# shehryar-malik/icrl

Hardware: AMD Instinct MI355X
Metric: env-steps/sec (ICRL outer loop, HCWithPos-v0) (higher is better)
Workload: dtype f32

## Files before the change

icrl_amd/_lib.py:

```python
import ctypes
import os

_HERE = os.path.dirname(os.path.abspath(__file__))
LIB_PATH = os.environ.get("ICRL_HIP_LIB") or os.path.join(_HERE, "lib", "libicrl_hip.so")

_lib = None
PPO_SPLIT_BYTES = 2560 * 1024

c_void_p, c_int, c_double, c_float = ctypes.c_void_p, ctypes.c_int, ctypes.c_double, ctypes.c_float

SIGNATURES = {
    "icrl_abi_version": [],
    "icrl_last_error": [],
    "icrl_clear_error": [],
    "icrl_gae_dual": [c_void_p] * 12 + [c_int, c_int] + [c_double] * 4 + [c_void_p],
    "icrl_gae_dual_ex": [c_void_p] * 12 + [c_int, c_int] + [c_double] * 4 + [c_int, c_void_p],
    "icrl_gae_dual_ws": [c_void_p] * 12 + [c_int, c_int] + [c_double] * 4 + [c_int, c_void_p, ctypes.c_longlong, c_void_p],
    "icrl_gae_dual_ws_bytes": [c_int, c_int],
    "icrl_policy_prepare": [c_void_p, c_void_p],
    "icrl_costnet_prepare": [c_void_p, c_void_p],
    "icrl_policy_forward": [c_void_p, c_void_p, c_void_p, c_int, c_int] + [c_void_p] * 8,
    "icrl_policy_evaluate": [c_void_p, c_void_p, c_void_p, c_int] + [c_void_p] * 5,
    "icrl_sample_episodes": [c_void_p] * 6 + [c_int] * 4 + [c_void_p, c_int] + [c_void_p] * 6,
    "icrl_cost_mlp_forward": [c_void_p, c_void_p, c_void_p, c_int, c_void_p, c_void_p],
# ... 16 lines not shown
    "icrl_ppo_lag_train": [c_void_p] * 11,
    "icrl_ppo_generic_row_floats": [c_void_p],
    "icrl_cn_prepare": [c_void_p, c_void_p, c_void_p, c_int, c_void_p, c_void_p],
    "icrl_cn_train_work_floats": [c_int, c_int, c_int, c_int],
    "icrl_cn_train": [c_void_p] * 6 + [c_int, c_int, c_void_p, c_void_p, c_int, c_void_p, c_void_p, c_void_p, c_void_p],
    "icrl_debug_rollout_profile": [c_void_p],
    "icrl_debug_rollout_profile_wide": [c_void_p],
    "icrl_debug_rollout_trace_wide": [c_void_p, c_int],
    "icrl_debug_stream_ref": [c_void_p] * 9 + [c_int, c_int, c_int, c_void_p],
    "icrl_minibatch_gather": [c_void_p, c_void_p, c_int] + [c_void_p] * 10,
    "icrl_adv_stats": [c_void_p, c_void_p, c_int, c_void_p, c_void_p],
    "icrl_ppo_lag_loss_fwd_bwd": [c_void_p] * 13 + [c_int] + [c_void_p] * 6,
    "icrl_clip_adam_step": [c_void_p] * 5 + [ctypes.c_longlong, c_void_p, c_void_p, c_void_p, c_void_p],
    "icrl_explained_variance": [c_void_p] * 4 + [ctypes.c_longlong, c_void_p, c_void_p, c_void_p],
    "icrl_dual_step": [c_void_p, c_void_p, c_void_p, c_float, c_float, c_float, c_float, c_void_p, c_void_p],
    "icrl_buffer_add": [c_void_p, c_int] + [c_void_p] * 13,
    "icrl_is_weights": [c_void_p, c_void_p, c_int, c_void_p, c_int, c_float, c_int, c_void_p, c_void_p, c_void_p, c_void_p],
    "icrl_cn_loss_fwd_bwd": [c_void_p, c_void_p, c_void_p, c_int, c_int, c_float, c_float, c_int, c_void_p, c_void_p, c_void_p, c_void_p],
    "icrl_cn_train_minibatch": [c_void_p] * 6 + [c_int, c_int, c_void_p, c_void_p, c_int, c_void_p, c_void_p, c_int, c_void_p,
                                c_void_p, c_void_p],
    "icrl_rollout_collect_batch": [c_int, c_void_p, c_void_p, c_void_p] + [c_double] * 4 + [c_int, c_void_p, ctypes.c_longlong, c_void_p],
    "icrl_gae_dual_batch": [c_int, c_void_p, c_int, c_int] + [c_double] * 4 + [c_void_p, ctypes.c_longlong, c_void_p],
    "icrl_sample_episodes_batch": [c_int, c_void_p, c_void_p, c_void_p] + [c_int] * 4 + [c_void_p, ctypes.c_longlong, c_void_p],
    "icrl_cn_train_batch": [c_int, c_void_p, c_void_p, ctypes.c_longlong, c_void_p],
    "icrl_ppo_lag_train_batch": [c_int, c_void_p, c_void_p, ctypes.c_longlong, c_void_p],
}
BATCH_ARGS_BYTES = 1024
RESTYPES = {"icrl_cn_train_work_floats": ctypes.c_size_t, "icrl_monitor_ws_bytes": ctypes.c_size_t, "icrl_host_step_ws_bytes": ctypes.c_size_t, "icrl_gae_dual_ws_bytes": ctypes.c_size_t, "icrl_last_error": ctypes.c_char_p, "icrl_clear_error": None}


class HipExtensionMissing(RuntimeError):
    pass


def lib():
    global _lib
    if _lib is None:
        import torch
        if not os.path.exists(LIB_PATH):
            raise HipExtensionMissing(
                f"{LIB_PATH} not built: run `python -c 'import __graft_entry__ as g; g.build()'` "
                "(or `make -C icrl_amd/csrc`). icrl_amd has no CPU fallback.")
        _lib = ctypes.CDLL(LIB_PATH)
        for name, argtypes in SIGNATURES.items():
            fn = getattr(_lib, name)
            fn.argtypes = argtypes
            fn.restype = RESTYPES.get(name, c_int)
    return _lib


byref = ctypes.byref
# ... 22 lines not shown
```

icrl_amd/csrc/rollout.hip:

```cpp
#include <stdio.h>
#include <stdlib.h>

#include "common.h"
#include "cost_fn.h"
#include "generic.h"

namespace icrl {

__global__ void policy_transpose_kernel(PolLayout L, const float* __restrict__ p, float* __restrict__ pt) {
  for (int i = blockIdx.x * blockDim.x + threadIdx.x; i < L.n; i += gridDim.x * blockDim.x) {
    int dst = i;
    for (int w = 0; w < 3; ++w) {
      if (i >= L.W1[w] && i < L.b1[w]) { int r = i - L.W1[w]; int j = r / L.O, k = r % L.O; dst = L.W1[w] + k * L.H1 + j; }
      if (i >= L.W2[w] && i < L.b2[w]) { int r = i - L.W2[w]; int j = r / L.H1, k = r % L.H1; dst = L.W2[w] + k * L.H2 + j; }
    }
    if (i >= L.Wa && i < L.ba) { int r = i - L.Wa; int a = r / L.H2, j = r % L.H2; dst = L.Wa + j * L.A + a; }
    pt[dst] = p[i];
  }
}

__global__ void costnet_transpose_kernel(CnLayout L, const float* __restrict__ p, float* __restrict__ pt) {
  for (int i = blockIdx.x * blockDim.x + threadIdx.x; i < L.n; i += gridDim.x * blockDim.x) {
    int dst = i;
    if (i >= L.W0 && i < L.b0) { int r = i - L.W0; int j = r / L.in, k = r % L.in; dst = L.W0 + k * L.H1 + j; }
// ... 2686 lines not shown
    if (i == 0) e.t_ep[n] = 0;
  }
}

struct SampleArgs {
  icrl_env_t env;
  icrl_norm_t nm;
  PolLayout pl;
  const float* PT;
  int pt_in_lds;
  const float* noise;
  const float* alow;
  const float* ahigh;
  int episodes_per_stream, rows_per_stream, deterministic, do_reset;
  const int* stream_row0;
  int total_rows;
  double* orig_obs;
  double* obs;
  float* actions;
  double* ep_rewards;
  int* ep_lengths;
};

template <int OCT>
__device__ __forceinline__ void sample_episodes_body(const SampleArgs& a) {
  __shared__ ActShared sh;
  PolRegs<OCT> R;
  load_pol_regs<OCT>(a.pl, a.PT, R);
  __shared__ int s_done;
  __shared__ double s_rew;
  __shared__ double Bl[MAX_OBS * MAX_ACT];
  __shared__ float noise_s[MAX_ACT], alow_s[MAX_ACT], ahigh_s[MAX_ACT];
  const int n = blockIdx.x, tid = threadIdx.x, lane = tid & 63;
  const int w = __builtin_amdgcn_readfirstlane(tid >> 6);
  const int O = a.pl.O, A = a.pl.A;
  const int AS = a.pl.discrete ? 1 : A;
  icrl_env_t env = a.env; globalize(env);
  const float* const noise_g = as_global(a.noise);
  float* const actions_g = as_global(a.actions);
  double* const orig_obs_g = as_global(a.orig_obs);
  double* const obs_g = as_global(a.obs);
  const int norm_obs = a.nm.norm_obs, deterministic = a.deterministic;
  const double clip_obs = a.nm.clip_obs;
  for (int i = tid; i < O * a.env.act_dim; i += 192) Bl[i] = a.env.B[i];
  env.B = Bl;
  const bool has_box = a.alow != nullptr && a.ahigh != nullptr;
  if (tid < MAX_ACT) { alow_s[tid] = (has_box && tid < A) ? a.alow[tid] : 0.f; ahigh_s[tid] = (has_box && tid < A) ? a.ahigh[tid] : 0.f; }
  const uint32_t e_key = a.env.key[n];
  uint32_t e_ctr = a.env.step_count[n];
  int e_tep = a.env.t_ep[n];
  double n_mean = 0.0, n_den = 1.0;
  if (tid < O && a.nm.norm_obs) { n_mean = a.nm.obs_mean[tid]; n_den = sqrt(a.nm.obs_var[tid] + a.nm.epsilon); }
  for (int i = tid; i < MAX_OBS; i += 192) sh.x[i] = 0.f;
  if (tid < O) {
    double v = a.env.s[(size_t)n * O + tid];
    if (a.do_reset) v = env_reset_value(a.env, e_key, e_ctr, tid);
    sh.s_new[tid] = v;
  }
  if (a.do_reset) e_tep = 0;
  __syncthreads();
  size_t row = a.stream_row0 != nullptr ? (size_t)a.stream_row0[n] : (size_t)n * a.rows_per_stream;
  const size_t row_end = a.stream_row0 != nullptr ? (size_t)a.total_rows : row + a.rows_per_stream;
  float noise_reg = (noise_g != nullptr && tid < AS) ? noise_g[row * AS + tid] : 0.f;
  for (int ep = 0; ep < a.episodes_per_stream; ++ep) {
    double ep_rew = 0.0;
    int ep_len = 0;
    while (true) {
      if (tid < O) {
        const double raw = sh.s_new[tid];
        double o = raw;
        if (norm_obs) o = fmin(fmax((raw - n_mean) / n_den, -clip_obs), clip_obs);
        sh.s_old[tid] = raw;
        sh.x[tid] = (float)o;
      }
      if (noise_g != nullptr && tid < AS) {
        noise_s[tid] = noise_reg;
        if (row + 1 < row_end) noise_reg = noise_g[(row + 1) * AS + tid];
      }
      __syncthreads();
      policy_forward_block<OCT>(a.pl, R, sh, noise_g ? noise_s : nullptr, deterministic || noise_g == nullptr,
                                has_box ? alow_s : nullptr, has_box ? ahigh_s : nullptr);
      __syncthreads();
      const bool in_rows = row < row_end;
      if (w == 0) {
        double rew; int done;
        env_step_wave(env, n, sh.s_old, sh.act_clip, e_key, e_ctr, e_tep, sh.s_new, rew, done);
        if (lane == 0) { s_done = done; s_rew = rew; }
        if (lane < AS && in_rows) actions_g[row * AS + lane] = sh.act_clip[lane];
      }
      __syncthreads();
      if (tid < O && in_rows) {
        const double raw = sh.s_new[tid];
        double o = raw;
        if (norm_obs) o = fmin(fmax((raw - n_mean) / n_den, -clip_obs), clip_obs);
        orig_obs_g[row * O + tid] = raw;
        obs_g[row * O + tid] = o;
      }
      ep_rew += s_rew;
      ++ep_len;
      ++row;
      const int done = s_done;
      __syncthreads();
      if (done) break;
    }
    if (tid == 0) { a.ep_rewards[(size_t)n * a.episodes_per_stream + ep] = ep_rew; a.ep_lengths[(size_t)n * a.episodes_per_stream + ep] = ep_len; }
  }
}

template <int OCT>
__global__ void __launch_bounds__(192) sample_episodes_kernel(SampleArgs a) {
  sample_episodes_body<OCT>(a);
}

template <int OCT>
__global__ void __launch_bounds__(192) sample_episodes_batch_kernel(const SampleArgs* __restrict__ runs) {
  __shared__ SampleArgs a;
  {
    const unsigned* src = reinterpret_cast<const unsigned*>(runs + blockIdx.y);
    unsigned* dst = reinterpret_cast<unsigned*>(&a);
    for (unsigned i = threadIdx.x; i < sizeof(SampleArgs) / 4; i += 192) dst[i] = src[i];
  }
  __syncthreads();
  sample_episodes_body<OCT>(a);
}

struct HostStepArgs {
  ActStepArgs act;
  icrl_norm_t nm;
  icrl_host_step_t hs;
  int N;
};

__host__ __device__ inline size_t host_copy_doubles(int N, int O) { return (size_t)2 * O + 7 + (size_t)3 * N; }
struct HostCopy {
  double *mean, *var, *count, *ret_stats, *cost_stats, *ret, *cost_ret, *cost;
  __device__ HostCopy(double* base, int N, int O)
      : mean(base), var(base + O), count(base + 2 * O), ret_stats(base + 2 * O + 1), cost_stats(base + 2 * O + 4),
        ret(base + 2 * O + 7), cost_ret(base + 2 * O + 7 + N), cost(base + 2 * O + 7 + 2 * N) {}
};

template <int OCT, int CIT>
__global__ void __launch_bounds__(256) host_step_kernel(HostStepArgs h, int k) {
  __shared__ ActShared sh;
  __shared__ double vec[2][128], dev2[2][128], ret_s[128], cret_s[128], rawr_s[128];
  __shared__ float rawc_s[128];
  __shared__ double dens[2];
// ... 462 lines not shown
                                          void* args_ws, long long args_ws_bytes, void* stream) {
  static_assert(sizeof(SampleArgs) <= ICRL_BATCH_ARGS_BYTES, "ICRL_BATCH_ARGS_BYTES");
  if (n_runs < 1 || n_runs > 65535) return fail("icrl_sample_episodes_batch: n_runs = %d (1..65535)", n_runs);
  if (args_ws == nullptr || args_ws_bytes < (long long)n_runs * ICRL_BATCH_ARGS_BYTES)
    return fail("icrl_sample_episodes_batch: args_ws holds %lld B, %d runs need %lld", args_ws_bytes, n_runs, (long long)n_runs * ICRL_BATCH_ARGS_BYTES);
  hipStream_t s = (hipStream_t)stream;
  SampleArgs* d_args = (SampleArgs*)args_ws;
  const icrl_sample_job_t& j0 = jobs[0];
  for (int r = 0; r < n_runs; ++r) {
    const icrl_sample_job_t& j = jobs[r];
    if (j.env->n_envs != j0.env->n_envs || j.env->obs_dim != j0.env->obs_dim || j.pol->act_dim != j0.pol->act_dim ||
        j.pol->discrete != j0.pol->discrete || j.env->max_steps != j0.env->max_steps)
      return fail("icrl_sample_episodes_batch: run %d differs from run 0 in a shape (streams / obs / act / discrete / max_steps)", r);
    SampleArgs a;
    const int bad = make_sample_args(j.env, j.nm, j.pol, j.noise, action_low, action_high, episodes_per_stream, rows_per_stream,
                                     deterministic, do_reset, j.stream_row0, j.total_rows, j.orig_obs, j.obs, j.actions, j.ep_rewards,
                                     j.ep_lengths, a);
    if (bad) return bad;
    const int e = put_args(a, d_args + r, s);
    if (e) return e;
  }
  if (j0.pol->obs_dim <= 32) hipLaunchKernelGGL(sample_episodes_batch_kernel<2>, dim3(j0.env->n_envs, n_runs), dim3(192), 0, s, d_args);
  else hipLaunchKernelGGL(sample_episodes_batch_kernel<8>, dim3(j0.env->n_envs, n_runs), dim3(192), 0, s, d_args);
  return (int)hipGetLastError();
}

extern "C" int icrl_cost_fn_rows(const icrl_cost_fn_t* cf, const double* obs, const float* acs, int N, float* cost, void* stream) {
  if (cf == nullptr || cf->n_hidden != ICRL_COST_FN) return fail("icrl_cost_fn_rows: not an analytic cost descriptor (n_hidden must be ICRL_COST_FN)");
  if (int e = cost_fn_check("icrl_cost_fn_rows", cf, 0, 0, -1)) return e;
  if (N <= 0 || cost == nullptr) return fail("icrl_cost_fn_rows: N = %d rows, cost = %p", N, (void*)cost);
  const bool wall = cf->kind == ICRL_COST_WALL_BEHIND || cf->kind == ICRL_COST_WALL_INFRONT || cf->kind == ICRL_COST_WALL_BOTH;
  if ((wall && obs == nullptr) || ((cf->kind == ICRL_COST_TORQUE || cf->kind == ICRL_COST_ACTION_EQUALS) && acs == nullptr))
    return fail("icrl_cost_fn_rows: cost kind %d reads the %s, which is NULL", cf->kind, wall ? "observations" : "actions");
  const int grid = (N + 255) / 256 < 1024 ? (N + 255) / 256 : 1024;
  hipLaunchKernelGGL(cost_fn_rows_kernel, dim3(grid), dim3(256), 0, (hipStream_t)stream, *cf, obs, acs, N, cost);
  return (int)hipGetLastError();
}

extern "C" int icrl_cost_mlp_forward(const icrl_costnet_t* cn, const double* obs, const float* acs, int N, float* cost,
                                     void* stream) {
  if (const icrl_cost_fn_t* cf = as_cost_fn(cn)) return icrl_cost_fn_rows(cf, obs, acs, N, cost, stream);
  if (N <= 0) return fail("cost forward: N = %d rows", N);
  if (costnet_is_wide(cn)) return launch_cn_cost_rows(cn, obs, acs, N, cost, 0, (hipStream_t)stream);
  if (!cn_ok(cn)) return bad_cn("cost forward", cn);
  CnLayout L = make_cn_layout(cn->in_dim, cn->n_hidden, cn->h1, cn->h2);
  if (cn->in_dim <= 32) hipLaunchKernelGGL(cost_forward_kernel<2>, dim3(N), dim3(64), 0, (hipStream_t)stream, *cn, L, obs, acs, N, cost, 0);
// ... 672 lines not shown
```

icrl_amd/icrl.py:

```python
import argparse
import json
import os
import sys
import time
import types

import numpy as np
import torch

from . import distributed as D, logger, utils
from .constraint_net import ConstraintNet
from .ppo_lag import PPOLagrangian
from .true_constraint_net import get_true_cost_function, mean_cost, null_cost
from .vec_env import VecNormalize, sync_envs_normalization
from . import envs, spaces


def setup(config):
    rank, world = getattr(config, "rank", 0), getattr(config, "world_size", 1)
    dev = config.device if str(config.device).startswith("cuda") else "cuda"
    envs.import_modules(getattr(config, "env_module", None))
    train_env = utils.make_train_env(env_id=config.train_env_id, save_dir=config.save_dir, use_cost_wrapper=True,
                                     base_seed=config.seed, num_threads=config.num_threads,
                                     normalize_obs=not config.dont_normalize_obs, normalize_reward=not config.dont_normalize_reward,
# ... 83 lines not shown
    st["rms_prev"] = D.allreduce_state([pol.params, pol.exp_avg, pol.exp_avg_sq, cn.params, cn.exp_avg, cn.exp_avg_sq],
                                       st["rms_list"], st["rms_prev"], st["world"], scalars=scal, force_collective=force)
    pol.prepare(); cn.prepare()
    if ev is not None:
        ev[1].record(); st["sync_events"].append(ev); st["sync_host_ms"].append(1e3 * (time.perf_counter() - t0))


def outer_iteration(st, itr):
    config, rank, world = st["config"], st["rank"], st["world"]
    train_env, sampling_env, eval_env, constraint_net = st["train_env"], st["sampling_env"], st["eval_env"], st["constraint_net"]
    if config.reset_policy and itr != 0:
        old_agent = st["agent"]
        st["agent"] = st["create_nominal_agent"]()
        if hasattr(old_agent, "_train_ws"):
            st["agent"]._train_ws = old_agent._train_ws
    nominal_agent = st["agent"]
    current_progress_remaining = 1 - float(itr) / float(config.n_iters)
    nominal_agent.learn(total_timesteps=config.forward_timesteps, cost_function="cost")
    forward_metrics = dict(logger.Logger.CURRENT.name_to_value)
    st["timesteps"] += nominal_agent.num_timesteps
    sync_envs_normalization(train_env, sampling_env)
    streams = getattr(config, "streams", None)
    A = 1 if nominal_agent.policy.discrete else nominal_agent.policy.act_dim
    orig_observations, observations, actions, rewards, lengths = utils.sample_from_agent(
        nominal_agent, sampling_env, config.expert_rollouts,
        noise=None if streams is None else streams.sample_noise(config.expert_rollouts * sampling_env.unwrapped.max_steps, A))
    mean, var = None, None
    if config.cn_normalize:
        mean, var = sampling_env.obs_rms.mean, sampling_env.obs_rms.var
    cn_perms = None
    if constraint_net.batch_size is not None and streams is not None and hasattr(streams, "cn_permutations"):
        cn_perms = streams.cn_permutations(config.backward_iters, min(int(orig_observations.shape[0]), int(np.asarray(constraint_net.expert_obs).shape[0])))
    backward_metrics = constraint_net.train(config.backward_iters, orig_observations, actions, lengths, mean, var,
                                            current_progress_remaining, perms=cn_perms)
    train_env.set_cost_function(constraint_net.cost_function)
    synchronise(st)
    average_true_cost = mean_cost(st["true_cost_function"], orig_observations, actions)
    samples_behind = float((orig_observations[..., 0] < -3).double().mean().item())
    samples_infront = float((orig_observations[..., 0] > 3).double().mean().item())
    sync_envs_normalization(train_env, eval_env)
    average_true_reward, std_true_reward = utils.evaluate_policy(
        nominal_agent, eval_env, n_eval_episodes=10, deterministic=False,
        noise=None if streams is None else streams.eval_noise(10 * eval_env.unwrapped.max_steps, A))
    forward_kl = reverse_kl = float("nan")
    if st["expert_agent"] is not None:
        forward_kl = utils.compute_kl(nominal_agent, st["d_expert_obs"], st["d_expert_acs"], st["expert_agent"])
        reverse_kl = utils.compute_kl(st["expert_agent"], orig_observations, actions, nominal_agent)
    best = st["best"]
    if config.save_dir and itr % config.save_every == 0 and rank == 0:
        path = os.path.join(config.save_dir, f"models/icrl_{itr}_itrs")
        os.makedirs(path, exist_ok=True)
        nominal_agent.save(os.path.join(path, "nominal_agent"))
        torch.save(nominal_agent.policy.state_dict(), os.path.join(path, "nominal_agent_policy.pth"))
        constraint_net.save(os.path.join(path, "cn.pt"))
        train_env.save(os.path.join(path, f"{itr}_train_env_stats.pkl"))
    if average_true_reward > best["reward"] and config.save_dir and rank == 0:
        nominal_agent.save(os.path.join(config.save_dir, "best_nominal_model"))
        torch.save(nominal_agent.policy.state_dict(), os.path.join(config.save_dir, "best_nominal_model_policy.pth"))
        constraint_net.save(os.path.join(config.save_dir, "best_cn_model.pt"))
        train_env.save(os.path.join(config.save_dir, "train_env_stats.pkl"))
    best["reward"] = max(best["reward"], average_true_reward)
    best["cost"] = min(best["cost"], average_true_cost)
    best["fkl"] = min(best["fkl"], forward_kl) if forward_kl == forward_kl else best["fkl"]
    best["rkl"] = min(best["rkl"], reverse_kl) if reverse_kl == reverse_kl else best["rkl"]
    metrics = {"time(m)": (time.time() - st["start_time"]) / 60, "iteration": itr, "timesteps": st["timesteps"],
               "true/reward": average_true_reward, "true/reward_std": std_true_reward, "true/cost": average_true_cost,
# ... 105 lines not shown
```

icrl_amd/structs.py:

```python
import ctypes as C

i32, f64, vp = C.c_int32, C.c_double, C.c_void_p


class EnvT(C.Structure):
    _fields_ = [("n_envs", i32), ("obs_dim", i32), ("act_dim", i32), ("max_steps", i32), ("reward_form", i32),
                ("wall_terminate", i32), ("broken", i32), ("_pad", i32),
                ("B", vp), ("s", vp), ("t_ep", vp), ("step_count", vp), ("key", vp)]


class NormT(C.Structure):
    _fields_ = [("training", i32), ("norm_obs", i32), ("norm_reward", i32), ("norm_cost", i32),
                ("clip_obs", f64), ("clip_reward", f64), ("clip_cost", f64), ("reward_gamma", f64), ("cost_gamma", f64),
                ("epsilon", f64),
                ("obs_mean", vp), ("obs_var", vp), ("obs_count", vp), ("ret_stats", vp), ("cost_stats", vp),
                ("ret", vp), ("cost_ret", vp)]


class PolicyT(C.Structure):
    _fields_ = [("obs_dim", i32), ("act_dim", i32), ("h1", i32), ("h2", i32), ("discrete", i32), ("n_params", i32),
                ("params", vp), ("params_t", vp), ("arch", vp)]


class CostNetT(C.Structure):
# ... 47 lines not shown
                ("adam_eps", C.c_float)]


class CnHyperT(C.Structure):
    _fields_ = [("iterations", i32), ("importance_sampling", i32), ("per_step", i32), ("gail", i32),
                ("reg_coeff", C.c_float), ("eps", C.c_float), ("target_kl_old_new", C.c_float), ("target_kl_new_old", C.c_float),
                ("lr", C.c_float), ("adam_beta1", C.c_float), ("adam_beta2", C.c_float), ("adam_eps", C.c_float)]


class RolloutJobT(C.Structure):
    _fields_ = [("env", vp), ("nm", vp), ("pol", vp), ("cn", vp), ("buf", vp), ("ag", vp), ("noise", vp)]


class GaeJobT(C.Structure):
    _fields_ = [(k, vp) for k in ("rewards", "costs", "reward_values", "cost_values", "dones", "last_v_r", "last_v_c", "last_dones",
                                  "adv_r", "adv_c", "ret_r", "ret_c", "ws")] + [("ws_bytes", C.c_longlong)]


class SampleJobT(C.Structure):
    _fields_ = ([(k, vp) for k in ("env", "nm", "pol", "noise", "stream_row0")] + [("total_rows", i32), ("_pad", i32)] +
                [(k, vp) for k in ("orig_obs", "obs", "actions", "ep_rewards", "ep_lengths")])


class CnTrainJobT(C.Structure):
    _fields_ = [("cn", vp), ("exp_avg", vp), ("exp_avg_sq", vp), ("adam_step", vp), ("nominal", vp), ("expert", vp), ("Nn", i32), ("Ne", i32),
                ("ep_offsets", vp), ("row_episode", vp), ("n_ep", i32), ("_pad", i32), ("hp", vp), ("work", vp), ("metrics", vp)]


class PpoTrainJobT(C.Structure):
    _fields_ = [(k, vp) for k in ("pol", "exp_avg", "exp_avg_sq", "adam_step", "buf", "perms", "nu", "hp", "stats", "sync_ws")]


def addr(struct):
    return C.addressof(struct) if struct is not None else None


def p(t):
    if t is None:
        return None
    assert t.is_contiguous()
    return t.data_ptr()

GAE_WS_BYTES = 256 * (256 * 8 + 4) + 64
```

icrl_amd/utils.py:

```python
import io
import os
import pickle
import types
import zipfile

import numpy as np
import torch

from . import _lib, spaces
from .policies import ActorTwoCriticsPolicy
from .structs import EnvT, HostEpisodeT, p
from . import envs
from .vec_env import ENV_IDS, DummyVecEnv, HipSynthVecEnv, HostVecEnv, SubprocVecEnv, VecCostWrapper, VecNormalize, VecNormalizeWithCost


def make_vec_env(env_id, n_envs, seed, device="cuda", env_index_offset=0, dummy_vec_env=False):
    if env_id in ENV_IDS:
        return HipSynthVecEnv.make(env_id, n_envs, seed, device, env_index_offset=env_index_offset)
    fns = [envs.spec(env_id)] * n_envs
    cls = DummyVecEnv if dummy_vec_env else SubprocVecEnv
    venv = cls(fns, device=device, env_index_offset=env_index_offset)
    venv.seed(seed)
    return venv


def make_train_env(env_id, save_dir, use_cost_wrapper, base_seed=0, num_threads=1, normalize_obs=True, normalize_reward=True,
                   normalize_cost=True, env_index_offset=0, device="cuda", **kwargs):
    import random
    random.seed(base_seed); np.random.seed(base_seed); torch.manual_seed(base_seed)
    env = make_vec_env(env_id, num_threads, base_seed, device, env_index_offset, dummy_vec_env=kwargs.pop("dummy_vec_env", False))
    if use_cost_wrapper:
        env = VecCostWrapper(env)
    if normalize_reward and normalize_cost:
        assert all(key in kwargs for key in ["cost_info_str", "reward_gamma", "cost_gamma"])
# ... 93 lines not shown
            lengths = self.out["ep_lengths"].cpu().numpy()
        lengths = np.asarray(lengths).astype(np.int64)
        if self.n_streams > 1:
            implied = np.concatenate([[0], np.cumsum(lengths)[:-1]])
            if not np.array_equal(implied, self.starts):
                if self.passes >= self.MAX_PASSES:
                    self.n_streams = 1
                    self.starts = np.zeros(1, np.int64)
                else:
                    self.starts = implied
                return False
        senv, env, dev = self.senv, self.env, self.dev
        total = int(lengths.sum())
        senv.step_count.fill_(int(np.uint32((self.base + total) & 0xFFFFFFFF).view(np.int32)))
        senv.s.copy_(self.st["s"][-1:]); senv.t_ep.zero_()
        env.old_obs = senv.s
        self.lengths = lengths
        self.keep = None if total == self.rows else total
        return True

    def rows_of(self, name):
        x = self.out[name]
        return x if self.keep is None else x[:self.keep]


class SteppedEpisodeRun:

    def __init__(self, agent, env, n_episodes, deterministic, noise):
        assert env.num_envs == 1, "You must pass only one environment when using this function"
        pol, senv = agent.policy, env.unwrapped
        dev, max_steps = senv.device, senv.max_steps
        A = 1 if pol.discrete else pol.act_dim
        rows = n_episodes * max_steps
        if noise is None and not deterministic:
            noise = torch.rand(rows, device=dev) if pol.discrete else torch.randn(rows, A, device=dev)
        if noise is not None:
            noise = torch.as_tensor(noise, device=dev).float().reshape(rows, -1).contiguous()
        was_training = env.training
        env.training = False
        try:
            orig, obs_l, acts, ep_rewards, lengths = [], [], [], [], []
            k, obs = 0, env.reset()
            for _ in range(n_episodes):
                done, ep_r, ep_l = False, 0.0, 0
                while not done:
                    actions, _, _, _ = pol.forward(obs, deterministic=deterministic, noise=None if noise is None else noise[k:k + 1])
# ... 92 lines not shown
                done = bool(d[0])
                launch(k, int(not (done and ep == n_episodes - 1)))
            ep_rewards.append(ep_r); lengths.append(ep_l)
        last_raw = out["orig_obs"][k - 1:k]
        henv.s.copy_(last_raw)
        nenv.old_obs, nenv.old_reward = last_raw.clone(), torch.full((1,), rew, dtype=torch.float64, device=dev)
        nenv.ret.zero_()
        if cw is not None:
            cw.previous_obs = last_raw.clone()
            cw.actions = out["actions"][k - 1:k].clone()
            if cw.cost_function is not None:
                nenv.cost_ret.zero_()
        out["ep_rewards"] = torch.as_tensor(np.asarray(ep_rewards, np.float64), device=dev)
        out["ep_lengths"] = torch.as_tensor(np.asarray(lengths, np.int32), device=dev)
        self.out, self._keepalive = out, (noise, lo, hi)
        self.lengths = np.asarray(lengths, np.int64)
        self.keep = None if k == rows else k

    def rows_of(self, name):
        x = self.out[name]
        return x if self.keep is None else x[:self.keep]


def _run_episodes(agent, env, n_episodes, deterministic, noise, parallel):
    if isinstance(env.unwrapped, HostVecEnv):
        if env.unwrapped.max_steps is None:
            raise ValueError("sampling / evaluation over a host env needs its episode limit: register it with max_episode_steps "
                             "(or give the env spec.max_episode_steps / _max_episode_steps)")
        if host_episodes_ok(agent, env):
            return HostEpisodeRun(agent, env, n_episodes, deterministic, noise)
        return SteppedEpisodeRun(agent, env, n_episodes, deterministic, noise)
    run = EpisodeRun(agent, env, n_episodes, deterministic, noise, parallel).prepare()
    run.launch()
    while not run.finish():
        run.prepare().launch()
    return run


def sample_from_agent(agent, env, rollouts, noise=None, parallel=True):
    return sample_result(_run_episodes(agent, env, rollouts, False, noise, parallel))


def sample_result(run, ep_rewards=None):
    return (run.rows_of("orig_obs"), run.rows_of("obs"), run.rows_of("actions"),
            run.out["ep_rewards"].cpu().numpy() if ep_rewards is None else np.asarray(ep_rewards), run.lengths)


def evaluate_policy(model, env, n_eval_episodes=10, deterministic=True, render=False, callback=None, reward_threshold=None,
                    return_episode_rewards=False, noise=None):
    run = _run_episodes(model, env, n_eval_episodes, deterministic, noise, parallel=False)
    return evaluate_result(run, None, reward_threshold, return_episode_rewards)


def evaluate_result(run, ep_rewards=None, reward_threshold=None, return_episode_rewards=False):
    ep_rewards = run.out["ep_rewards"].cpu().numpy() if ep_rewards is None else np.asarray(ep_rewards)
    if return_episode_rewards:
        return list(ep_rewards), list(run.lengths)
    mean_reward, std_reward = float(np.mean(ep_rewards)), float(np.std(ep_rewards))
    if reward_threshold is not None:
        assert mean_reward > reward_threshold
    return mean_reward, std_reward


def compute_kl(agent_2, observations, actions, agent_1=None):
    return float(compute_kl_device(agent_2, observations, actions, agent_1).item())


def compute_kl_device(agent_2, observations, actions, agent_1=None):
    kl = -agent_2.policy.evaluate_actions(observations, actions)[1].reshape(-1)
    if agent_1 is not None:
        kl = kl + agent_1.policy.evaluate_actions(observations, actions)[1].reshape(-1)
    return kl.sum() / kl.shape[0]

# ... 121 lines not shown
```

include/icrl_hip.h:

```cpp
#ifndef ICRL_HIP_H
#define ICRL_HIP_H

#include <stdint.h>

#ifdef __cplusplus
extern "C" {
#endif


typedef struct {
  int32_t n_envs, obs_dim, act_dim, max_steps;
  int32_t reward_form;
  int32_t wall_terminate;
  int32_t broken;
  int32_t _pad;
  const double* B;
  double* s;
  int32_t* t_ep;
  uint32_t* step_count;
  const uint32_t* key;
} icrl_env_t;

typedef struct {
  int32_t training, norm_obs, norm_reward, norm_cost;
// ... 247 lines not shown
  void* ws;
  long long ws_bytes;
} icrl_gae_job_t;
int icrl_gae_dual_batch(int n_runs, const icrl_gae_job_t* jobs, int T, int N, double reward_gamma, double reward_gae_lambda,
                        double cost_gamma, double cost_gae_lambda, void* args_ws, long long args_ws_bytes, void* stream);

typedef struct {
  const icrl_env_t* env;
  const icrl_norm_t* nm;
  const icrl_policy_t* pol;
  const float* noise;
  const int32_t* stream_row0;
  int32_t total_rows, _pad;
  double *orig_obs, *obs;
  float* actions;
  double* ep_rewards;
  int32_t* ep_lengths;
} icrl_sample_job_t;
int icrl_sample_episodes_batch(int n_runs, const icrl_sample_job_t* jobs, const float* action_low, const float* action_high,
                               int episodes_per_stream, int rows_per_stream, int deterministic, int do_reset,
                               void* args_ws, long long args_ws_bytes, void* stream);

typedef struct {
  const icrl_costnet_t* cn;
  float *exp_avg, *exp_avg_sq;
  int32_t* adam_step;
  const float *nominal, *expert;
  int32_t Nn, Ne;
  const int32_t *ep_offsets, *row_episode;
  int32_t n_ep, _pad;
  const icrl_cn_hyper_t* hp;
  float *work, *metrics;
} icrl_cn_train_job_t;
int icrl_cn_train_batch(int n_runs, const icrl_cn_train_job_t* jobs, void* args_ws, long long args_ws_bytes, void* stream);

typedef struct {
  const icrl_policy_t* pol;
  float *exp_avg, *exp_avg_sq;
  int32_t* adam_step;
  const icrl_buffer_t* buf;
  const int32_t* perms;
  const float* nu;
  const icrl_ppo_hyper_t* hp;
  float* stats;
  void* sync_ws;
} icrl_ppo_train_job_t;
// ... 51 lines not shown
```

Before: 936,200.

## Run sequential episodes speculatively in parallel with chained predecessor validation

Adds a chained episode sampler that launches one workgroup per episode. Each workgroup speculatively guesses its starting RNG counter and row offset, then re-runs if its predecessor publishes a different end position, so episodes that used to run one after another can overlap. Finished rows are compacted from per-stream slots into the contiguous output. Expert sampling and evaluation are also fused into a single launch. The cost is extra spin-waiting, possible redundant recomputation, a requirement that every workgroup be co-resident, and a new workspace allocation on each call.

Result: faster. 947,300, median of 6 (+1.2%).

```diff
diff --git a/icrl_amd/_lib.py b/icrl_amd/_lib.py
--- a/icrl_amd/_lib.py
+++ b/icrl_amd/_lib.py
@@ -62,11 +62,13 @@
     "icrl_rollout_collect_batch": [c_int, c_void_p, c_void_p, c_void_p] + [c_double] * 4 + [c_int, c_void_p, ctypes.c_longlong, c_void_p],
     "icrl_gae_dual_batch": [c_int, c_void_p, c_int, c_int] + [c_double] * 4 + [c_void_p, ctypes.c_longlong, c_void_p],
     "icrl_sample_episodes_batch": [c_int, c_void_p, c_void_p, c_void_p] + [c_int] * 4 + [c_void_p, ctypes.c_longlong, c_void_p],
+    "icrl_sample_episodes_chain_ws_bytes": [c_int, c_void_p],
+    "icrl_sample_episodes_chain": [c_int, c_void_p, c_void_p, c_void_p, c_int, c_void_p, ctypes.c_longlong, c_void_p, ctypes.c_longlong, c_void_p],
     "icrl_cn_train_batch": [c_int, c_void_p, c_void_p, ctypes.c_longlong, c_void_p],
     "icrl_ppo_lag_train_batch": [c_int, c_void_p, c_void_p, ctypes.c_longlong, c_void_p],
 }
 BATCH_ARGS_BYTES = 1024
-RESTYPES = {"icrl_cn_train_work_floats": ctypes.c_size_t, "icrl_monitor_ws_bytes": ctypes.c_size_t, "icrl_host_step_ws_bytes": ctypes.c_size_t, "icrl_gae_dual_ws_bytes": ctypes.c_size_t, "icrl_last_error": ctypes.c_char_p, "icrl_clear_error": None}
+RESTYPES = {"icrl_cn_train_work_floats": ctypes.c_size_t, "icrl_monitor_ws_bytes": ctypes.c_size_t, "icrl_host_step_ws_bytes": ctypes.c_size_t, "icrl_gae_dual_ws_bytes": ctypes.c_size_t, "icrl_sample_episodes_chain_ws_bytes": ctypes.c_size_t, "icrl_last_error": ctypes.c_char_p, "icrl_clear_error": None}
 
 
 class HipExtensionMissing(RuntimeError):
diff --git a/icrl_amd/csrc/rollout.hip b/icrl_amd/csrc/rollout.hip
--- a/icrl_amd/csrc/rollout.hip
+++ b/icrl_amd/csrc/rollout.hip
@@ -2732,13 +2732,27 @@
   int* ep_lengths;
 };
 
-template <int OCT>
-__device__ __forceinline__ void sample_episodes_body(const SampleArgs& a) {
+struct ChainArgs {
+  SampleArgs s;
+  unsigned* next_start;
+  unsigned* status;
+  int* exec_steps;
+  double* slot_orig;
+  double* slot_obs;
+  float* slot_act;
+  const int* base_count;
+  int fixed_len, n_streams;
+};
+constexpr unsigned CHAIN_UNSET = 0xFFFFFFFEu;
+
+template <int OCT, bool CHAIN = false>
+__device__ __forceinline__ void sample_episodes_body(const SampleArgs& a, const ChainArgs* c = nullptr) {
   __shared__ ActShared sh;
   PolRegs<OCT> R;
   load_pol_regs<OCT>(a.pl, a.PT, R);
   __shared__ int s_done;
   __shared__ double s_rew;
+  __shared__ unsigned s_word;
   __shared__ double Bl[MAX_OBS * MAX_ACT];
   __shared__ float noise_s[MAX_ACT], alow_s[MAX_ACT], ahigh_s[MAX_ACT];
   const int n = blockIdx.x, tid = threadIdx.x, lane = tid & 63;
@@ -2747,9 +2761,9 @@
   const int AS = a.pl.discrete ? 1 : A;
   icrl_env_t env = a.env; globalize(env);
   const float* const noise_g = as_global(a.noise);
-  float* const actions_g = as_global(a.actions);
-  double* const orig_obs_g = as_global(a.orig_obs);
-  double* const obs_g = as_global(a.obs);
+  float* const actions_g = as_global(CHAIN ? c->slot_act : a.actions);
+  double* const orig_obs_g = as_global(CHAIN ? c->slot_orig : a.orig_obs);
+  double* const obs_g = as_global(CHAIN ? c->slot_obs : a.obs);
   const int norm_obs = a.nm.norm_obs, deterministic = a.deterministic;
   const double clip_obs = a.nm.clip_obs;
   for (int i = tid; i < O * a.env.act_dim; i += 192) Bl[i] = a.env.B[i];
@@ -2762,20 +2776,38 @@
   double n_mean = 0.0, n_den = 1.0;
   if (tid < O && a.nm.norm_obs) { n_mean = a.nm.obs_mean[tid]; n_den = sqrt(a.nm.obs_var[tid] + a.nm.epsilon); }
   for (int i = tid; i < MAX_OBS; i += 192) sh.x[i] = 0.f;
+  const int max_steps = a.env.max_steps;
+  unsigned* const words = CHAIN ? as_global(c->next_start) : nullptr;
+  const uint32_t base = CHAIN ? (uint32_t)as_global(c->base_count)[0] : 0u;
+  const size_t slot0 = CHAIN ? (size_t)n * max_steps : 0;
+  unsigned pos = CHAIN ? (unsigned)n * (unsigned)max_steps : 0u;
+  bool validated = !CHAIN || n == 0 || c->fixed_len != 0;
+  int executed = 0;
+  bool again;
+  do {
+  again = false;
+  if (CHAIN) {
+    __syncthreads();
+    e_ctr = base + pos;
+    if (n > 0 || a.do_reset) e_tep = 0;
+    if (tid == 0 && !c->fixed_len) xstore(words + n, (pos + (unsigned)max_steps) << 1);
+  }
   if (tid < O) {
     double v = a.env.s[(size_t)n * O + tid];
-    if (a.do_reset) v = env_reset_value(a.env, e_key, e_ctr, tid);
+    if (a.do_reset || (CHAIN && n > 0)) v = env_reset_value(a.env, e_key, e_ctr, tid);
     sh.s_new[tid] = v;
   }
-  if (a.do_reset) e_tep = 0;
+  if (!CHAIN && a.do_reset) e_tep = 0;
   __syncthreads();
-  size_t row = a.stream_row0 != nullptr ? (size_t)a.stream_row0[n] : (size_t)n * a.rows_per_stream;
-  const size_t row_end = a.stream_row0 != nullptr ? (size_t)a.total_rows : row + a.rows_per_stream;
+  size_t row = CHAIN ? (size_t)pos : a.stream_row0 != nullptr ? (size_t)a.stream_row0[n] : (size_t)n * a.rows_per_stream;
+  const size_t row_end = (CHAIN || a.stream_row0 != nullptr) ? (size_t)a.total_rows : row + a.rows_per_stream;
   float noise_reg = (noise_g != nullptr && tid < AS) ? noise_g[row * AS + tid] : 0.f;
   for (int ep = 0; ep < a.episodes_per_stream; ++ep) {
     double ep_rew = 0.0;
     int ep_len = 0;
     while (true) {
+      unsigned word = CHAIN_UNSET;
+      if (CHAIN && !validated && tid == 128) word = xload(words + n - 1);
       if (tid < O) {
         const double raw = sh.s_new[tid];
         double o = raw;
@@ -2791,30 +2823,76 @@
       policy_forward_block<OCT>(a.pl, R, sh, noise_g ? noise_s : nullptr, deterministic || noise_g == nullptr,
                                 has_box ? alow_s : nullptr, has_box ? ahigh_s : nullptr);
       __syncthreads();
-      const bool in_rows = row < row_end;
+      const bool in_rows = CHAIN || row < row_end;
+      const size_t orow = CHAIN ? slot0 + (size_t)ep_len : row;
       if (w == 0) {
         double rew; int done;
         env_step_wave(env, n, sh.s_old, sh.act_clip, e_key, e_ctr, e_tep, sh.s_new, rew, done);
         if (lane == 0) { s_done = done; s_rew = rew; }
-        if (lane < AS && in_rows) actions_g[row * AS + lane] = sh.act_clip[lane];
-      }
+        if (lane < AS && in_rows) actions_g[orow * AS + lane] = sh.act_clip[lane];
+      }
+      if (CHAIN && tid == 128) s_word = word;
       __syncthreads();
       if (tid < O && in_rows) {
         const double raw = sh.s_new[tid];
         double o = raw;
         if (norm_obs) o = fmin(fmax((raw - n_mean) / n_den, -clip_obs), clip_obs);
-        orig_obs_g[row * O + tid] = raw;
-        obs_g[row * O + tid] = o;
+        orig_obs_g[orow * O + tid] = raw;
+        obs_g[orow * O + tid] = o;
       }
       ep_rew += s_rew;
       ++ep_len;
       ++row;
       const int done = s_done;
+      if (CHAIN) {
+        ++executed;
+        const unsigned pw = s_word;
+        if (!validated && pw != CHAIN_UNSET) {
+          if ((pw >> 1) != pos) { pos = pw >> 1; again = true; }
+          validated = (pw & 1u) != 0u;
+        }
+      }
       __syncthreads();
+      if (CHAIN && again) break;
       if (done) break;
     }
-    if (tid == 0) { a.ep_rewards[(size_t)n * a.episodes_per_stream + ep] = ep_rew; a.ep_lengths[(size_t)n * a.episodes_per_stream + ep] = ep_len; }
-  }
+    if (CHAIN) {
+      if (again) break;
+      if (tid == 0 && !validated) xstore(words + n, (pos + (unsigned)ep_len) << 1);
+      for (int spins = 0; !validated && !again; ++spins) {
+        if (spins == (1 << 22)) {
+          if (tid == 0) { atomicOr(as_global(c->status), 1u); a.ep_lengths[n] = -1; }
+          return;
+        }
+        if (tid == 0) s_word = xload(words + n - 1);
+        __syncthreads();
+        const unsigned pw = s_word;
+        if (pw != CHAIN_UNSET) {
+          if ((pw >> 1) != pos) { pos = pw >> 1; again = true; }
+          validated = (pw & 1u) != 0u;
+        }
+        __syncthreads();
+        if (!validated && !again) __builtin_amdgcn_s_sleep(32);
+      }
+      if (again) break;
+      if (tid == 0) {
+        a.ep_rewards[n] = ep_rew; a.ep_lengths[n] = ep_len;
+        if (c->exec_steps != nullptr) c->exec_steps[n] = executed;
+        if (!c->fixed_len) xstore(words + n, ((pos + (unsigned)ep_len) << 1) | 1u);
+      }
+      if (!c->fixed_len) {
+        const size_t nd = (size_t)ep_len * O, na = (size_t)ep_len * AS;
+        const double* so = orig_obs_g + slot0 * O; const double* sn = obs_g + slot0 * O; const float* sa = actions_g + slot0 * AS;
+        double* dorig = as_global(a.orig_obs) + (size_t)pos * O; double* dobs = as_global(a.obs) + (size_t)pos * O;
+        float* dact = as_global(a.actions) + (size_t)pos * AS;
+#pragma unroll 4
+        for (size_t i = tid; i < nd; i += 192) { dorig[i] = so[i]; dobs[i] = sn[i]; }
+#pragma unroll 4
+        for (size_t i = tid; i < na; i += 192) dact[i] = sa[i];
+      }
+    } else if (tid == 0) { a.ep_rewards[(size_t)n * a.episodes_per_stream + ep] = ep_rew; a.ep_lengths[(size_t)n * a.episodes_per_stream + ep] = ep_len; }
+  }
+  } while (CHAIN && again);
 }
 
 template <int OCT>
@@ -2832,6 +2910,24 @@
   }
   __syncthreads();
   sample_episodes_body<OCT>(a);
+}
+
+template <int OCT>
+__global__ void __launch_bounds__(192) sample_episodes_chain_kernel(const ChainArgs* __restrict__ jobs) {
+  __shared__ ChainArgs c;
+  {
+    const unsigned* src = reinterpret_cast<const unsigned*>(jobs + blockIdx.y);
+    unsigned* dst = reinterpret_cast<unsigned*>(&c);
+    for (unsigned i = threadIdx.x; i < sizeof(ChainArgs) / 4; i += 192) dst[i] = src[i];
+  }
+  __syncthreads();
+  if ((int)blockIdx.x >= c.n_streams) return;
+  sample_episodes_body<OCT, true>(c.s, &c);
+}
+
+__global__ void __launch_bounds__(64) chain_prep_kernel(ChainArgs v, ChainArgs* dst, int clear_status) {
+  if (threadIdx.x == 0) { *dst = v; if (clear_status) *v.status = 0u; }
+  for (int i = threadIdx.x; i < v.n_streams; i += 64) v.next_start[i] = CHAIN_UNSET;
 }
 
 struct HostStepArgs {
@@ -3340,6 +3436,84 @@
   }
   if (j0.pol->obs_dim <= 32) hipLaunchKernelGGL(sample_episodes_batch_kernel<2>, dim3(j0.env->n_envs, n_runs), dim3(192), 0, s, d_args);
   else hipLaunchKernelGGL(sample_episodes_batch_kernel<8>, dim3(j0.env->n_envs, n_runs), dim3(192), 0, s, d_args);
+  return (int)hipGetLastError();
+}
+
+static size_t chain_align(size_t b) { return (b + 255) / 256 * 256; }
+static size_t chain_slot_bytes(const icrl_chain_job_t& j) {
+  if (j.fixed_len) return 0;
+  const size_t rows = (size_t)j.env->n_envs * j.env->max_steps;
+  const size_t AS = j.pol->discrete ? 1 : j.pol->act_dim;
+  return 2 * chain_align(rows * j.env->obs_dim * sizeof(double)) + chain_align(rows * AS * sizeof(float));
+}
+static int chain_total_streams(int n_jobs, const icrl_chain_job_t* jobs) {
+  long long t = 0;
+  for (int r = 0; r < n_jobs; ++r) t += jobs[r].env->n_envs > 0 ? jobs[r].env->n_envs : 0;
+  return t > (1 << 30) ? (1 << 30) : (int)t;
+}
+
+extern "C" size_t icrl_sample_episodes_chain_ws_bytes(int n_jobs, const icrl_chain_job_t* jobs) {
+  if (n_jobs < 1 || jobs == nullptr) return 0;
+  size_t b = 256 + chain_align((size_t)chain_total_streams(n_jobs, jobs) * sizeof(unsigned));
+  for (int r = 0; r < n_jobs; ++r) b += chain_slot_bytes(jobs[r]);
+  return b;
+}
+
+extern "C" int icrl_sample_episodes_chain(int n_jobs, const icrl_chain_job_t* jobs, const float* action_low, const float* action_high,
+                                          int do_reset, void* ws, long long ws_bytes, void* args_ws, long long args_ws_bytes, void* stream) {
+  static_assert(sizeof(ChainArgs) <= ICRL_BATCH_ARGS_BYTES, "ICRL_BATCH_ARGS_BYTES");
+  if (n_jobs < 1 || n_jobs > 65535 || jobs == nullptr) return fail("icrl_sample_episodes_chain: n_jobs = %d (1..65535)", n_jobs);
+  static int n_cu = 0;
+  if (n_cu == 0) {
+    int dev = 0;
+    if (hipGetDevice(&dev) != hipSuccess || hipDeviceGetAttribute(&n_cu, hipDeviceAttributeMultiprocessorCount, dev) != hipSuccess) n_cu = 0;
+  }
+  const int total = chain_total_streams(n_jobs, jobs);
+  if (total > n_cu)
+    return fail("icrl_sample_episodes_chain: refused: %d streams on %d compute units (every stream must be resident while its successors wait)", total, n_cu);
+  int max_streams = 0;
+  for (int r = 0; r < n_jobs; ++r) {
+    const icrl_chain_job_t& j = jobs[r];
+    if (policy_is_wide(j.pol)) return fail("icrl_sample_episodes_chain: refused: job %d has a generic-shape policy", r);
+    if (j.episodes_per_stream != 1) return fail("icrl_sample_episodes_chain: refused: job %d runs %d episodes per stream (1 only)", r, j.episodes_per_stream);
+    if ((j.pol->obs_dim <= 32) != (jobs[0].pol->obs_dim <= 32)) return fail("icrl_sample_episodes_chain: refused: job %d and job 0 take different kernels (obs %d / %d)", r, j.pol->obs_dim, jobs[0].pol->obs_dim);
+    if (j.env->n_envs < 1 || j.base_count == nullptr) return fail("icrl_sample_episodes_chain: job %d: %d streams, base_count %p", r, j.env->n_envs, (const void*)j.base_count);
+    if ((long long)j.env->n_envs * j.env->max_steps >= (1ll << 31) - 1) return fail("icrl_sample_episodes_chain: job %d: %d streams x %d steps do not fit a 31-bit row", r, j.env->n_envs, j.env->max_steps);
+    if (j.env->n_envs > max_streams) max_streams = j.env->n_envs;
+  }
+  const long long need = (long long)icrl_sample_episodes_chain_ws_bytes(n_jobs, jobs);
+  if (ws == nullptr || ws_bytes < need) return fail("icrl_sample_episodes_chain: ws holds %lld B, the jobs need %lld", ws_bytes, need);
+  if (args_ws == nullptr || args_ws_bytes < (long long)n_jobs * ICRL_BATCH_ARGS_BYTES)
+    return fail("icrl_sample_episodes_chain: args_ws holds %lld B, %d jobs need %lld", args_ws_bytes, n_jobs, (long long)n_jobs * ICRL_BATCH_ARGS_BYTES);
+  hipStream_t s = (hipStream_t)stream;
+  ChainArgs* d_args = (ChainArgs*)args_ws;
+  char* const base = (char*)ws;
+  unsigned* words = (unsigned*)(base + 256);
+  char* slots = base + 256 + chain_align((size_t)total * sizeof(unsigned));
+  for (int r = 0; r < n_jobs; ++r) {
+    const icrl_chain_job_t& j = jobs[r];
+    const int rows = j.env->n_envs * j.env->max_steps;
+    ChainArgs c;
+    const int bad = make_sample_args(j.env, j.nm, j.pol, j.noise, action_low, action_high, 1, j.env->max_steps, j.deterministic, do_reset, nullptr,
+                                     rows, j.orig_obs, j.obs, j.actions, j.ep_rewards, j.ep_lengths, c.s);
+    if (bad) return bad;
+    c.next_start = words; words += j.env->n_envs;
+    c.status = (unsigned*)base;
+    c.exec_steps = j.exec_steps;
+    c.base_count = j.base_count;
+    c.fixed_len = j.fixed_len != 0; c.n_streams = j.env->n_envs;
+    if (c.fixed_len) { c.slot_orig = j.orig_obs; c.slot_obs = j.obs; c.slot_act = j.actions; }
+    else {
+      const size_t AS = j.pol->discrete ? 1 : j.pol->act_dim;
+      const size_t ob = chain_align((size_t)rows * j.env->obs_dim * sizeof(double));
+      c.slot_orig = (double*)slots; c.slot_obs = (double*)(slots + ob); c.slot_act = (float*)(slots + 2 * ob);
+      slots += 2 * ob + chain_align((size_t)rows * AS * sizeof(float));
+    }
+    hipLaunchKernelGGL(chain_prep_kernel, dim3(1), dim3(64), 0, s, c, d_args + r, (int)(r == 0));
+    if (const int e = (int)hipGetLastError()) return e;
+  }
+  if (jobs[0].pol->obs_dim <= 32) hipLaunchKernelGGL(sample_episodes_chain_kernel<2>, dim3(max_streams, n_jobs), dim3(192), 0, s, d_args);
+  else hipLaunchKernelGGL(sample_episodes_chain_kernel<8>, dim3(max_streams, n_jobs), dim3(192), 0, s, d_args);
   return (int)hipGetLastError();
 }
 
diff --git a/icrl_amd/icrl.py b/icrl_amd/icrl.py
--- a/icrl_amd/icrl.py
+++ b/icrl_amd/icrl.py
@@ -129,9 +129,18 @@
     sync_envs_normalization(train_env, sampling_env)
     streams = getattr(config, "streams", None)
     A = 1 if nominal_agent.policy.discrete else nominal_agent.policy.act_dim
-    orig_observations, observations, actions, rewards, lengths = utils.sample_from_agent(
-        nominal_agent, sampling_env, config.expert_rollouts,
-        noise=None if streams is None else streams.sample_noise(config.expert_rollouts * sampling_env.unwrapped.max_steps, A))
+    draws_cn_perms = constraint_net.batch_size is not None and streams is not None and hasattr(streams, "cn_permutations")
+    fused = (world <= 1 and not getattr(config, "force_collective", False) and not draws_cn_perms and utils.chain_enabled()
+             and utils.episodes_fusable(sampling_env, eval_env))
+    sample_noise = None if streams is None else streams.sample_noise(config.expert_rollouts * sampling_env.unwrapped.max_steps, A)
+    if fused:
+        sync_envs_normalization(train_env, eval_env)
+        (orig_observations, observations, actions, rewards, lengths), (average_true_reward, std_true_reward) = utils.sample_and_evaluate(
+            nominal_agent, sampling_env, config.expert_rollouts, eval_env, n_eval_episodes=10, deterministic=False, sample_noise=sample_noise,
+            eval_noise=None if streams is None else streams.eval_noise(10 * eval_env.unwrapped.max_steps, A))
+    else:
+        orig_observations, observations, actions, rewards, lengths = utils.sample_from_agent(
+            nominal_agent, sampling_env, config.expert_rollouts, noise=sample_noise)
     mean, var = None, None
     if config.cn_normalize:
         mean, var = sampling_env.obs_rms.mean, sampling_env.obs_rms.var
@@ -145,10 +154,11 @@
     average_true_cost = mean_cost(st["true_cost_function"], orig_observations, actions)
     samples_behind = float((orig_observations[..., 0] < -3).double().mean().item())
     samples_infront = float((orig_observations[..., 0] > 3).double().mean().item())
-    sync_envs_normalization(train_env, eval_env)
-    average_true_reward, std_true_reward = utils.evaluate_policy(
-        nominal_agent, eval_env, n_eval_episodes=10, deterministic=False,
-        noise=None if streams is None else streams.eval_noise(10 * eval_env.unwrapped.max_steps, A))
+    if not fused:
+        sync_envs_normalization(train_env, eval_env)
+        average_true_reward, std_true_reward = utils.evaluate_policy(
+            nominal_agent, eval_env, n_eval_episodes=10, deterministic=False,
+            noise=None if streams is None else streams.eval_noise(10 * eval_env.unwrapped.max_steps, A))
     forward_kl = reverse_kl = float("nan")
     if st["expert_agent"] is not None:
         forward_kl = utils.compute_kl(nominal_agent, st["d_expert_obs"], st["d_expert_acs"], st["expert_agent"])
diff --git a/icrl_amd/structs.py b/icrl_amd/structs.py
--- a/icrl_amd/structs.py
+++ b/icrl_amd/structs.py
@@ -93,6 +93,12 @@
                 [(k, vp) for k in ("orig_obs", "obs", "actions", "ep_rewards", "ep_lengths")])
 
 
+class ChainJobT(C.Structure):
+    _fields_ = ([(k, vp) for k in ("env", "nm", "pol", "noise", "base_count")] +
+                [("episodes_per_stream", i32), ("deterministic", i32), ("fixed_len", i32), ("_pad", i32)] +
+                [(k, vp) for k in ("orig_obs", "obs", "actions", "ep_rewards", "ep_lengths", "exec_steps")])
+
+
 class CnTrainJobT(C.Structure):
     _fields_ = [("cn", vp), ("exp_avg", vp), ("exp_avg_sq", vp), ("adam_step", vp), ("nominal", vp), ("expert", vp), ("Nn", i32), ("Ne", i32),
                 ("ep_offsets", vp), ("row_episode", vp), ("n_ep", i32), ("_pad", i32), ("hp", vp), ("work", vp), ("metrics", vp)]
diff --git a/icrl_amd/utils.py b/icrl_amd/utils.py
--- a/icrl_amd/utils.py
+++ b/icrl_amd/utils.py
@@ -9,7 +9,7 @@
 
 from . import _lib, spaces
 from .policies import ActorTwoCriticsPolicy
-from .structs import EnvT, HostEpisodeT, p
+from .structs import ChainJobT, EnvT, HostEpisodeT, addr, p
 from . import envs
 from .vec_env import ENV_IDS, DummyVecEnv, HipSynthVecEnv, HostVecEnv, SubprocVecEnv, VecCostWrapper, VecNormalize, VecNormalizeWithCost
 
@@ -149,6 +149,62 @@
     def rows_of(self, name):
         x = self.out[name]
         return x if self.keep is None else x[:self.keep]
+
+    def chain_ok(self):
+        return chain_enabled() and self.n_streams > 1 and self.n_streams == self.n_episodes and not self.pol.wide
+
+    def prepare_chain(self):
+        senv, dev, O, A, n = self.senv, self.dev, self.O, self.A, self.n_streams
+        self.eps_per, self.rows_per = 1, self.max_steps
+        self.st = dict(s=senv.s.repeat(n, 1).contiguous(), t_ep=senv.t_ep.repeat(n).contiguous(),
+                       step_count=torch.zeros(n, dtype=torch.int32, device=dev), key=senv.key.repeat(n).contiguous())
+        st = self.st
+        self.e = EnvT(n, O, senv.act_dim, self.max_steps, senv.reward_form, int(senv.wall_terminate), int(senv.broken), 0,
+                      p(senv.B), p(st["s"]), p(st["t_ep"]), p(st["step_count"]), p(st["key"]))
+        rows = self.rows
+        self.out = dict(orig_obs=torch.empty(rows, O, dtype=torch.float64, device=dev), obs=torch.empty(rows, O, dtype=torch.float64, device=dev),
+                        actions=torch.empty(rows, A, device=dev), ep_rewards=torch.empty(n, dtype=torch.float64, device=dev),
+                        ep_lengths=torch.empty(n, dtype=torch.int32, device=dev), exec_steps=torch.empty(n, dtype=torch.int32, device=dev))
+        out = self.out
+        self.job = ChainJobT(addr(self.e), addr(self.nm), addr(self.ps), p(self.noise), p(senv.step_count), 1, int(self.deterministic),
+                             int(self.fixed_len), 0, p(out["orig_obs"]), p(out["obs"]), p(out["actions"]), p(out["ep_rewards"]),
+                             p(out["ep_lengths"]), p(out["exec_steps"]))
+        self.passes += 1
+        return self
+
+    def finish_chain(self):
+        lengths = self.out["ep_lengths"].cpu().numpy().astype(np.int64)
+        if (lengths < 0).any():
+            raise RuntimeError("icrl_sample_episodes_chain: a stream gave up waiting for its predecessor (a workgroup was not resident)")
+        senv, env = self.senv, self.env
+        senv.step_count.copy_(self.st["step_count"][-1:])
+        senv.s.copy_(self.st["s"][-1:]); senv.t_ep.zero_()
+        env.old_obs = senv.s
+        total = int(lengths.sum())
+        self.lengths = lengths
+        self.keep = None if total == self.rows else total
+        return True
+
+
+def chain_enabled():
+    return os.environ.get("ICRL_EPISODE_CHAIN", "1") not in ("0",)
+
+
+def launch_chain(runs):
+    r0 = runs[0]
+    jobs = (ChainJobT * len(runs))(*[r.job for r in runs])
+    lib = _lib.lib()
+    ws_bytes = int(lib.icrl_sample_episodes_chain_ws_bytes(len(runs), jobs))
+    ws = torch.empty(ws_bytes, dtype=torch.uint8, device=r0.dev)
+    args = torch.empty(len(runs) * _lib.BATCH_ARGS_BYTES, dtype=torch.uint8, device=r0.dev)
+    try:
+        _lib.check(lib.icrl_sample_episodes_chain(len(runs), jobs, p(r0.lo), p(r0.hi), 1, p(ws), ws_bytes, p(args), args.numel(),
+                                                  _lib.current_stream()), "icrl_sample_episodes_chain")
+    except ValueError as err:
+        if "icrl_sample_episodes_chain: refused:" in str(err):
+            return False
+        raise
+    return True
 
 
 class SteppedEpisodeRun:
@@ -287,7 +343,7 @@
         return x if self.keep is None else x[:self.keep]
 
 
-def _run_episodes(agent, env, n_episodes, deterministic, noise, parallel):
+def _run_episodes(agent, env, n_episodes, deterministic, noise, parallel, chain=False):
     if isinstance(env.unwrapped, HostVecEnv):
         if env.unwrapped.max_steps is None:
             raise ValueError("sampling / evaluation over a host env needs its episode limit: register it with max_episode_steps "
@@ -295,15 +351,45 @@
         if host_episodes_ok(agent, env):
             return HostEpisodeRun(agent, env, n_episodes, deterministic, noise)
         return SteppedEpisodeRun(agent, env, n_episodes, deterministic, noise)
-    run = EpisodeRun(agent, env, n_episodes, deterministic, noise, parallel).prepare()
-    run.launch()
+    return _launch_and_finish(EpisodeRun(agent, env, n_episodes, deterministic, noise, parallel), chain)
+
+
+def _launch_and_finish(run, chain=True):
+    if chain and run.chain_ok() and launch_chain([run.prepare_chain()]):
+        run.finish_chain()
+        return run
+    run.passes = 0
+    run.prepare().launch()
     while not run.finish():
         run.prepare().launch()
     return run
 
 
+def _is_device_env(env):
+    return not isinstance(env.unwrapped, HostVecEnv)
+
+
+def episodes_fusable(sampling_env, eval_env):
+    return _is_device_env(sampling_env) and _is_device_env(eval_env) and sampling_env.unwrapped is not eval_env.unwrapped
+
+
+def sample_and_evaluate(agent, sampling_env, n_rollouts, eval_env, n_eval_episodes=10, deterministic=True, sample_noise=None,
+                        eval_noise=None, parallel=True, reward_threshold=None, return_episode_rewards=False):
+    if episodes_fusable(sampling_env, eval_env):
+        s_run = EpisodeRun(agent, sampling_env, n_rollouts, False, sample_noise, parallel)
+        e_run = EpisodeRun(agent, eval_env, n_eval_episodes, deterministic, eval_noise, False)
+        if s_run.chain_ok() and e_run.chain_ok() and launch_chain([s_run.prepare_chain(), e_run.prepare_chain()]):
+            s_run.finish_chain(); e_run.finish_chain()
+        else:
+            _launch_and_finish(s_run); _launch_and_finish(e_run)
+        return sample_result(s_run), evaluate_result(e_run, None, reward_threshold, return_episode_rewards)
+    return (sample_from_agent(agent, sampling_env, n_rollouts, sample_noise, parallel),
+            evaluate_policy(agent, eval_env, n_eval_episodes, deterministic, reward_threshold=reward_threshold,
+                            return_episode_rewards=return_episode_rewards, noise=eval_noise))
+
+
 def sample_from_agent(agent, env, rollouts, noise=None, parallel=True):
-    return sample_result(_run_episodes(agent, env, rollouts, False, noise, parallel))
+    return sample_result(_run_episodes(agent, env, rollouts, False, noise, parallel, chain=True))
 
 
 def sample_result(run, ep_rewards=None):
@@ -313,7 +399,7 @@
 
 def evaluate_policy(model, env, n_eval_episodes=10, deterministic=True, render=False, callback=None, reward_threshold=None,
                     return_episode_rewards=False, noise=None):
-    run = _run_episodes(model, env, n_eval_episodes, deterministic, noise, parallel=False)
+    run = _run_episodes(model, env, n_eval_episodes, deterministic, noise, parallel=False, chain=True)
     return evaluate_result(run, None, reward_threshold, return_episode_rewards)
 
 
diff --git a/include/icrl_hip.h b/include/icrl_hip.h
--- a/include/icrl_hip.h
+++ b/include/icrl_hip.h
@@ -293,6 +293,23 @@
                                void* args_ws, long long args_ws_bytes, void* stream);
 
 typedef struct {
+  const icrl_env_t* env;
+  const icrl_norm_t* nm;
+  const icrl_policy_t* pol;
+  const float* noise;
+  const int32_t* base_count;
+  int32_t episodes_per_stream, deterministic, fixed_len, _pad;
+  double *orig_obs, *obs;
+  float* actions;
+  double* ep_rewards;
+  int32_t* ep_lengths;
+  int32_t* exec_steps;
+} icrl_chain_job_t;
+size_t icrl_sample_episodes_chain_ws_bytes(int n_jobs, const icrl_chain_job_t* jobs);
+int icrl_sample_episodes_chain(int n_jobs, const icrl_chain_job_t* jobs, const float* action_low, const float* action_high, int do_reset,
+                               void* ws, long long ws_bytes, void* args_ws, long long args_ws_bytes, void* stream);
+
+typedef struct {
   const icrl_costnet_t* cn;
   float *exp_avg, *exp_avg_sq;
   int32_t* adam_step;
```
